# acrlabs/kube-scheduler-rs-reference

Hardware: AMD Instinct MI355X
Metric: pod x node predicate evals/s (higher is better)
Workload: dtype int64

## Files before the change

kube_scheduler_rs_reference_amd/csrc/kernels_build.hpp:

```cpp
#pragma once
#include <hip/hip_runtime.h>
#include <stdint.h>

#include "../../include/ksched.h"
#include "apply_admit.hpp"
#include "kernels_direct.hpp"
#include "tile_index.hpp"

namespace ksched {

struct BuildFitArgs {
    const int64_t *ncpu, *nmem;
    uint64_t *tables, *aux;
    const uint32_t *tile_list;
    const uint32_t *dirty;
    uint32_t n, rows, row_cpu;
};

__device__ __forceinline__ int64_t shfl_xor_key(int64_t x, uint32_t j) {
    const uint32_t lo = (uint32_t)__shfl_xor((int)(uint32_t)x, (int)j, 64), hi = (uint32_t)__shfl_xor((int)(uint32_t)((uint64_t)x >> 32), (int)j, 64);
    return (int64_t)(((uint64_t)hi << 32) | lo);
}
__device__ __forceinline__ uint32_t shfl_xor_key(uint32_t x, uint32_t j) { return (uint32_t)__shfl_xor((int)x, (int)j, 64); }

template <class K>
__device__ __forceinline__ void bitonic_sort_tile(K &kv, uint32_t &ki, K *s_key, uint16_t *s_idx, uint32_t i) {
    for (uint32_t k = 2; k <= (uint32_t)kTileNodes; k <<= 1) {
        for (uint32_t j = k >> 1; j > 0; j >>= 1) {
            K pv;
            uint32_t pi;
            if (j >= 64u) {
                s_key[i] = kv;
                s_idx[i] = (uint16_t)ki;
                __syncthreads();
                pv = s_key[i ^ j];
                pi = s_idx[i ^ j];
                __syncthreads();
            } else {
                pv = shfl_xor_key(kv, j);
                pi = shfl_xor_key(ki, j);
            }
            const bool ascending = (i & k) == 0u, lower = (i & j) == 0u;
            const bool p_less = pv < kv || (pv == kv && pi < ki);
            const bool take = (lower == ascending) ? p_less : !p_less;
            kv = take ? pv : kv;
            ki = take ? pi : ki;
        }
    }
    s_key[i] = kv;
    s_idx[i] = (uint16_t)ki;
    __syncthreads();
}

__global__ __launch_bounds__(1024) void k_build_tile_fit(const BuildFitArgs a) {
    kernarg_warm<sizeof(BuildFitArgs)>();
    __shared__ int64_t s_key[kTileNodes];
    __shared__ uint16_t s_idx[kTileNodes];
    __shared__ uint64_t s_wave[16];
    __shared__ uint64_t s_rows[kFitRows * kTileWords];
    const uint32_t tile = a.tile_list ? a.tile_list[blockIdx.x] : blockIdx.x;
    if (a.dirty && a.dirty[tile] != a.dirty[gridDim.x]) return;
    const uint32_t res = blockIdx.y;
    const int64_t *col = res == 0 ? a.ncpu : a.nmem;
    const uint32_t base = tile * kTileNodes;
    const uint32_t m = min((uint32_t)kTileNodes, a.n - base);
    const uint32_t i = threadIdx.x, lane = i & 63u, wave = i >> 6;
    int64_t kv = (i < m) ? col[base + i] : INT64_MAX;
    uint32_t ki = i;
    bitonic_sort_tile(kv, ki, s_key, s_idx, i);
    uint64_t *aux = a.aux + (size_t)tile * kAuxWords;
    {
        int64_t t;
        if (i == 0) {
            t = s_key[kTileNodes - 1];
        } else {
            const uint32_t L = 31u - (uint32_t)__builtin_clz(i), j = i - (1u << L);
            t = s_key[((2u * j + 1u) << (9u - L)) - 1u];
        }
        reinterpret_cast<int64_t *>(aux)[(size_t)res * kAuxTreeWords + i] = t;
    }
    {
        const bool live = ki < m;
        const uint32_t sub = ki / kSubNodes;
        const uint64_t x = live ? (1ull << (8u * sub)) : 0ull;
        uint64_t incl = x;
#pragma unroll
        for (uint32_t d = 1; d < 64; d <<= 1) {
            const uint32_t lo = (uint32_t)__shfl_up((int)(uint32_t)incl, d, 64), hi = (uint32_t)__shfl_up((int)(uint32_t)(incl >> 32), d, 64);
            if (lane >= d) incl += ((uint64_t)hi << 32) | lo;
        }
        if (lane == 63) s_wave[wave] = incl;
        __syncthreads();
        uint64_t before = 0, total = 0;
        for (uint32_t w = 0; w < 16; ++w) {
            const uint64_t t = s_wave[w];
            before += (w < wave) ? t : 0ull;
            total += t;
        }
        const uint64_t excl = before + incl - x;
        uint64_t *cnt = aux + 2u * kAuxTreeWords + (size_t)res * kCntEntries;
        cnt[i] = excl;
        if (i < (uint32_t)kCntEntries - (uint32_t)kTileNodes) cnt[kTileNodes + i] = total;
        __syncthreads();
        s_idx[i] = 0xFFFFu;
        __syncthreads();
        if (live) s_idx[sub * kSubNodes + (uint32_t)((excl >> (8u * sub)) & 0xFFull)] = (uint16_t)(ki & (kSubNodes - 1u));
    }
    __syncthreads();
    {
        const uint32_t sub = i >> 7, c = i & 127u;
        uint64_t *mine = s_rows + c * kTileWords + 2u * sub;
        const uint32_t node = s_idx[sub * kSubNodes + c];
        uint64_t lo = (node < 64u) ? (1ull << node) : 0ull, hi = (node >= 64u && node < 128u) ? (1ull << (node - 64u)) : 0ull;
        if (i < (uint32_t)kTileWords) s_rows[(kFitRows - 1) * kTileWords + i] = 0ull;
        auto shfl_down64 = [](uint64_t x, uint32_t d) -> uint64_t {
            const uint32_t l = (uint32_t)__shfl_down((int)(uint32_t)x, d, 64), h = (uint32_t)__shfl_down((int)(uint32_t)(x >> 32), d, 64);
            return ((uint64_t)h << 32) | l;
        };
#pragma unroll
        for (uint32_t d = 1; d < 64u; d <<= 1) {
            const uint64_t olo = shfl_down64(lo, d), ohi = shfl_down64(hi, d);
            if (lane + d < 64u) {
                lo |= olo;
                hi |= ohi;
            }
        }
        if ((c >> 6) == 1u && lane == 0) {
            s_wave[2u * sub] = lo;
            s_wave[2u * sub + 1u] = hi;
        }
        __syncthreads();
        if ((c >> 6) == 0u) {
            lo |= s_wave[2u * sub];
            hi |= s_wave[2u * sub + 1u];
        }
        mine[0] = lo;
        mine[1] = hi;
    }
    __syncthreads();
    uint64_t *T = a.tables + ((size_t)tile * a.rows + a.row_cpu + (size_t)res * kFitRows) * kTileWords;
    for (uint32_t k = i; k < (uint32_t)kFitRows * kTileWords; k += 1024u) T[k] = s_rows[k];
}

struct BuildListArgs {
    const uint32_t *nlab;
    uint8_t *lists;
    const uint32_t *tile_list;
    uint32_t n, nlist;
    uint32_t list_col[kMaxListKeys];
};
__global__ __launch_bounds__(1024) void k_build_tile_list(const BuildListArgs a) {
    kernarg_warm<sizeof(BuildListArgs)>();
    __shared__ uint32_t s_key[kTileNodes];
    __shared__ uint16_t s_idx[kTileNodes];
    const uint32_t tile = a.tile_list ? a.tile_list[blockIdx.x] : blockIdx.x, j = blockIdx.y, i = threadIdx.x;
    const uint32_t base = tile * kTileNodes;
    const uint32_t m = min((uint32_t)kTileNodes, a.n - base);
    uint32_t kv = (i < m) ? a.nlab[(size_t)a.list_col[j] * a.n + base + i] : 0u;
    uint32_t ki = i;
    bitonic_sort_tile(kv, ki, s_key, s_idx, i);
    uint8_t *L = a.lists + ((size_t)tile * a.nlist + j) * kListBytes;
    reinterpret_cast<uint32_t *>(L)[i] = kv;
    reinterpret_cast<uint16_t *>(L + kTileNodes * 4u)[i] = (uint16_t)ki;
}

struct BuildNamedArgs {
    const uint32_t *nlab;
    const uint64_t *ntaint;
    uint64_t *tables;
    const uint32_t *lab_meta;
    const uint32_t *tile_list;
    uint32_t n, rows, nkeys, ngroups, row_valid, row_taint, named_rows;
};


__global__ __launch_bounds__(1024) void k_build_tile_named(const BuildNamedArgs a) {
    kernarg_warm<sizeof(BuildNamedArgs)>();
    extern __shared__ __attribute__((aligned(16))) uint64_t s_named[];
    const uint32_t tile = a.tile_list ? a.tile_list[blockIdx.x] : blockIdx.x;
    const uint32_t base = tile * kTileNodes;
    const uint32_t m = min((uint32_t)kTileNodes, a.n - base);
    const uint32_t i = threadIdx.x, lane = i & 63u, wave = i >> 6;
    const bool live = i < m;
    const uint32_t total = a.named_rows * kTileWords;
    for (uint32_t k = i; k < total; k += 1024u) s_named[k] = 0ull;
    __syncthreads();
    {
        const uint64_t word = __ballot(live);
        if (lane == 0) s_named[a.row_valid * kTileWords + wave] = word;
    }
    if (a.ngroups) {
        const uint64_t t = (live && a.ntaint) ? a.ntaint[base + i] : 0ull;
        for (uint32_t g = 0; g < a.ngroups; ++g) {
            const uint32_t tg = (uint32_t)((t >> (4u * g)) & 15ull);
            for (uint32_t sset = 0; sset < 16; ++sset) {
                const uint64_t word = __ballot(live && (tg & ~sset) == 0u);
                if (lane == 0) s_named[(a.row_taint + 16u * g + sset) * kTileWords + wave] = word;
            }
        }
    }
    for (uint32_t k = 0; k < a.nkeys; ++k) {
        const uint32_t lb = a.lab_meta[k];
        if (lb == kLabList) continue;
        const uint32_t id = live ? a.nlab[(size_t)k * a.n + base + i] : 0u;
        if (id) atomicOr((unsigned long long *)&s_named[(size_t)(lb + id - 1u) * kTileWords + wave], 1ull << lane);
    }
    __syncthreads();
    uint64_t *T = a.tables + (size_t)tile * a.rows * kTileWords;
    for (uint32_t k = i; k < total; k += 1024u) T[k] = s_named[k];
}

constexpr uint32_t kPatchInline = 16;
struct PatchArgs {
    int64_t *ncpu, *nmem, *nrec;
    const uint32_t *idx;
    const int64_t *cpu, *mem;
    uint32_t count;
    uint32_t idx_in[kPatchInline];
    int64_t cpu_in[kPatchInline], mem_in[kPatchInline];
    uint32_t *tile_out;
    uint32_t ntiles;
    uint32_t tiles_in[kPatchInline];
};
__global__ __launch_bounds__(256) void k_patch_nodes(const PatchArgs a) {
    kernarg_warm<sizeof(PatchArgs)>();
    const uint32_t t = blockIdx.x * blockDim.x + threadIdx.x;
    if (t >= a.count) return;
    if (a.tile_out && t < a.ntiles) a.tile_out[t] = a.tiles_in[t];
    uint32_t node;
    int64_t c, m;
    if (a.idx) {
        node = a.idx[t];
        c = a.cpu[t];
        m = a.mem[t];
    } else {
        node = a.idx_in[t];
        c = a.cpu_in[t];
        m = a.mem_in[t];
    }
    a.ncpu[node] = c;
    a.nmem[node] = m;
    a.nrec[(size_t)kNodeRecWords * node] = c;
    a.nrec[(size_t)kNodeRecWords * node + 1] = m;
}

struct PatchLabelsArgs {
    uint32_t *nlab;
    uint64_t *ntaint;
    int64_t *nrec;
    const uint32_t *idx;
    const uint32_t *lab;
    const uint64_t *taints;
    uint32_t count, n, nkeys;
};
__global__ __launch_bounds__(256) void k_patch_labels(const PatchLabelsArgs a) {
    kernarg_warm<sizeof(PatchLabelsArgs)>();
    const uint32_t t = blockIdx.x * blockDim.x + threadIdx.x;
    if (t >= a.count) return;
    const uint32_t node = a.idx[t];
    uint32_t l[8];
#pragma unroll
    for (uint32_t k = 0; k < 8; ++k) l[k] = 0u;
    for (uint32_t k = 0; k < a.nkeys; ++k) {
        const uint32_t id = a.lab[(size_t)k * a.count + t];
        a.nlab[(size_t)k * a.n + node] = id;
        if (k < 8u) l[k] = id;
    }
    int64_t *r = a.nrec + (size_t)kNodeRecWords * node;
    if (a.taints) {
        const uint64_t tb = a.taints[t];
        a.ntaint[node] = tb;
        r[2] = (int64_t)tb;
    }
#pragma unroll
    for (uint32_t k = 0; k < 4; ++k) r[4 + k] = (int64_t)(((uint64_t)l[2 * k + 1] << 32) | l[2 * k]);
}

constexpr uint32_t kApplyUnclaimed = 0xFFFFFFFFu;
struct ApplyArgs {
    const int32_t *bindings;
    const int64_t *req_cpu, *req_mem;
    const uint8_t *ok;
    int32_t *status;
    uint64_t *acc;
    uint32_t *claim;
    uint8_t *ovf;
    uint32_t *dirty;
    int64_t *ncpu, *nmem, *nrec;
    uint32_t p, n, tiles, gen;
    uint32_t first_per_node, release;
    uint32_t row_lo;
    uint32_t sharded;
    const uint64_t *gathered;
    uint32_t nranks, rank;
};

__device__ __forceinline__ bool apply_eligible(const ApplyArgs &a, uint32_t i, int32_t b) {
    return b >= 0 && (uint32_t)b < a.n && (!a.ok || a.ok[i] != 0);
}

__global__ __launch_bounds__(256) void k_apply_claim(const ApplyArgs a) {
    for (uint32_t i = blockIdx.x * blockDim.x + threadIdx.x; i < a.p; i += gridDim.x * blockDim.x) {
        const int32_t b = a.bindings[i];
        if (apply_eligible(a, i, b)) atomicMin(a.claim + b, a.row_lo + i);
    }
}

__device__ __forceinline__ void acc_add(uint64_t *p, uint64_t v) {
    if (v) __hip_atomic_fetch_add(p, v, __ATOMIC_RELAXED, __HIP_MEMORY_SCOPE_AGENT);
}

__global__ __launch_bounds__(256) void k_apply_accumulate(const ApplyArgs a) {
    const uint32_t t0 = blockIdx.x * blockDim.x + threadIdx.x;
    if (t0 == 0 && !a.sharded) a.dirty[a.tiles] = a.gen;
    for (uint32_t i = t0; i < a.p; i += gridDim.x * blockDim.x) {
        const int32_t b = a.bindings[i];
        int32_t st;
        if (b < 0) {
            st = KSCHED_APPLY_UNBOUND;
        } else if ((uint32_t)b >= a.n) {
            st = KSCHED_APPLY_BAD_NODE;
        } else if (a.ok && a.ok[i] == 0) {
            st = KSCHED_APPLY_NOT_OK;
        } else if (a.first_per_node && a.claim[b] != a.row_lo + i) {
            st = KSCHED_APPLY_DEFERRED;
        } else {
// ... 364 lines not shown
```

kube_scheduler_rs_reference_amd/csrc/ksched_api.hip:

```cpp
#include "../../include/ksched.h"

#include <hip/hip_runtime.h>

#include <algorithm>
#include <cstdio>
#include <cstdlib>
#include <cstring>
#include <mutex>
#include <new>
#include <numeric>
#include <stdexcept>
#include <string>
#include <utility>
#include <vector>


#include "apply_plan.hpp"
#include "bestfit_layout.hpp"
#include "comm_rccl.hpp"
#include "eval_plan.hpp"
#include "eval_request.hpp"
#include "kernels_build.hpp"
#include "kernels_direct.hpp"
#include "kernels_fused.hpp"
#include "kernels_pick_uniform.hpp"
#include "kernels_summary.hpp"
#include "kernels_pick_spread.hpp"
#include "kernels_pick_pack.hpp"
#include "kernels_combine.hpp"
#include "kernels_combine_soft.hpp"
#include "kernels_selop.hpp"
#include "kernels_seltag.hpp"
#include "mask_alloc.hpp"
#include "merge_sort_plan.hpp"
#include "pipe_plan.hpp"
#include "snapshot_change.hpp"
#include "stream_order.hpp"
#include "tile_index.hpp"

using namespace ksched;

static_assert(kListBytes == 6144u && kTileNodes == 1024, "k_pick_bestfit_listed (kernels_direct.hpp) addresses the tile lists with these sizes");
static_assert(kChangeTileNodes == (uint32_t)kTileNodes, "snapshot_change.hpp lists the tiles an update touches");
static_assert(kApplyTileNodes == (uint32_t)kTileNodes && kApplyIdleClaim == kApplyUnclaimed, "apply_plan.hpp sizes the commit by the tile and bounds the global pod indexes by the idle claim");
static_assert(sizeof(BestfitRowsArgs::lvl_off) == 4 * kBfMaxLevels && sizeof(BfLevelsArgs::lvl_off) == 4 * kBfMaxLevels, "bestfit_layout.hpp sizes the level arrays the kernels carry");

namespace {

template <class T>
struct DevBuf {
    T *ptr = nullptr;
    size_t cap = 0;
    DevBuf() = default;
    DevBuf(DevBuf &&o) noexcept { *this = std::move(o); }
    DevBuf &operator=(DevBuf &&o) noexcept {
        std::swap(ptr, o.ptr);
        std::swap(cap, o.cap);
        return *this;
    }
    ~DevBuf() { release(); }
    void release() {
        if (ptr) (void)hipFree(ptr);
        ptr = nullptr;
        cap = 0;
    }
    hipError_t reserve(size_t n) {
        if (n <= cap) return hipSuccess;
        release();
        hipError_t e = hipMalloc((void **)&ptr, std::max<size_t>(n, 1) * sizeof(T));
        if (e == hipSuccess) cap = n;
        return e;
    }
};

struct SortScratch {
    DevBuf<int64_t> k0[2], k1[2];
    DevBuf<uint32_t> idx[2];
    bool holds(size_t n) const { return n <= k0[0].cap && n <= k0[1].cap && n <= idx[0].cap && n <= idx[1].cap; }
    hipError_t reserve(size_t n, bool second_key) {
        hipError_t e = hipSuccess;
        for (int b = 0; b < 2 && e == hipSuccess; ++b) {
            e = k0[b].reserve(n);
            if (e == hipSuccess && second_key) e = k1[b].reserve(n);
            if (e == hipSuccess) e = idx[b].reserve(n);
        }
        return e;
    }
};

struct BestfitIndex {
    DevBuf<uint32_t> bf_order, bf_rank;
    DevBuf<int64_t> bf_mem, bf_cpu;
    DevBuf<int64_t> cpu_sorted;
    DevBuf<uint32_t> by_cpu, cpurank;
    DevBuf<int64_t> samples;
    DevBuf<int64_t> levels;
    DevBuf<uint64_t> rows;
    SortScratch sort;
    DevBuf<uint32_t> handover;
    DevBuf<uint64_t> trace;
    BfOrderLayout order;
    BfRowLayout row;
    BfRotation rotation;
    bool rows_built = false;
    bool order_stale = true, rows_stale = false;

    hipError_t reserve_for(uint32_t n) {
        hipError_t e = bf_order.reserve(n);
        if (e == hipSuccess) e = bf_rank.reserve(n);
        if (e == hipSuccess) e = bf_mem.reserve(bf_searched_elems(n));
        if (e == hipSuccess) e = bf_cpu.reserve(n);
        if (e == hipSuccess) e = cpu_sorted.reserve(bf_searched_elems(n));
        return e;
    }
    void mark(Stale what) {
        if (stale_order(what)) order_stale = true;
        if (stale_rows_only(what)) rows_stale = true;
        if (what == Stale::kEverything) rows_built = false;
    }
    bool stale() const { return order_stale || rows_stale; }
};
// ... 223 lines not shown
    if (pl.carrier_waits_build)
        if (int rc = stream_wait_build(c, s)) return rc;
    if (!pl.record_callers) return KSCHED_OK;
    for (size_t i = 0; i < o.callers();) {
        if (hipEventRecord(o.caller_res(i).ev, hip_stream_of(o.caller(i))) != hipSuccess) {
            (void)hipGetLastError();
            const StreamRes gone = o.drop(i);
            (void)hipEventDestroy(gone.ev);
            continue;
        }
        HIPCHK(c, hipStreamWaitEvent(s, o.caller_res(i).ev, 0));
        ++i;
    }
    return KSCHED_OK;
}

int snapshot_end(ksched_ctx *c) {
    HIPCHK(c, hipEventRecord(c->ev_build, hip_stream_of(c->order.change_stream())));
    c->order.committed();
    return KSCHED_OK;
}

int apply_order_begin(ksched_ctx *c, hipStream_t hs) {
    if (!c->order.plan_apply(hs).change_waits_hs) return KSCHED_OK;
    if (!c->apply.ev) HIPCHK(c, hipEventCreateWithFlags(&c->apply.ev, hipEventDisableTiming));
    HIPCHK(c, hipEventRecord(c->apply.ev, hs));
    HIPCHK(c, hipStreamWaitEvent(hip_stream_of(c->order.change_stream()), c->apply.ev, 0));
    return KSCHED_OK;
}

int apply_order_end(ksched_ctx *c, hipStream_t hs) { return c->order.plan_apply(hs).hs_waits_change ? stream_wait_build(c, hs) : KSCHED_OK; }

struct SnapshotChange {
    ksched_ctx *c = nullptr;
    bool done = false;
    ~SnapshotChange() {
        if (c && !done) {
            c->have_nodes = false;
            c->apply.invalidate();
        }
    }
    int begin(ksched_ctx *ctx) {
        if (int rc = snapshot_begin(ctx)) return rc;
        c = ctx;
        return KSCHED_OK;
    }
    int stage(size_t bytes, size_t dev_bytes, uint8_t **h) {
        if (c->h_stage) HIPCHK(c, hipEventSynchronize(c->ev_stage));
        if (bytes > c->h_stage_cap) {
            if (c->h_stage) (void)hipHostFree(c->h_stage);
            c->h_stage = nullptr;
            c->h_stage_cap = 0;
            const size_t cap = std::max<size_t>(bytes + bytes / 4, 1u << 16);
            HIPCHK(c, hipHostMalloc((void **)&c->h_stage, cap, hipHostMallocDefault));
            c->h_stage_cap = cap;
        }
        *h = c->h_stage;
        HIPCHK(c, c->d_stage.reserve(dev_bytes));
        return KSCHED_OK;
    }
    int upload(size_t dev_bytes) {
        const hipStream_t s = change_stream(c);
        if (dev_bytes) HIPCHK(c, hipMemcpyAsync(c->d_stage.ptr, c->h_stage, dev_bytes, hipMemcpyHostToDevice, s));
        HIPCHK(c, hipEventRecord(c->ev_stage, s));
        return KSCHED_OK;
    }
    int commit(Stale what) {
        c->bestfit.mark(what);
        if (int rc = snapshot_end(c)) return rc;
        c->have_nodes = true;
        done = true;
        return KSCHED_OK;
    }
};


int launch_build_fit(ksched_ctx *c, const uint32_t *d_tile_list, uint32_t count, const uint32_t *d_dirty = nullptr) {
    const IndexedLayout &l = c->idx.lay;
    BuildFitArgs a{};
    a.ncpu = c->ncpu.ptr;
    a.nmem = c->nmem.ptr;
    a.tables = c->idx.d_tables;
    a.aux = c->idx.d_aux;
    a.tile_list = d_tile_list;
    a.dirty = d_tile_list ? nullptr : d_dirty;
    a.n = l.n;
    a.rows = l.rows;
    a.row_cpu = l.row_cpu;
    hipLaunchKernelGGL(k_build_tile_fit, dim3(d_tile_list ? count : l.tiles, 2), dim3(1024), 0, change_stream(c), a);
    HIPCHK(c, hipGetLastError());
    return KSCHED_OK;
}

int launch_build_lists(ksched_ctx *c, const uint32_t *d_tile_list = nullptr, uint32_t count = 0) {
    const IndexedLayout &l = c->idx.lay;
    if (l.nlist == 0) return KSCHED_OK;
    BuildListArgs a{};
    a.nlab = c->nlab.ptr;
    a.lists = c->idx.d_list;
    a.tile_list = d_tile_list;
    a.n = l.n;
    a.nlist = l.nlist;
    for (uint32_t j = 0; j < l.nlist; ++j) a.list_col[j] = l.list_col[j];
    hipLaunchKernelGGL(k_build_tile_list, dim3(d_tile_list ? count : l.tiles, l.nlist), dim3(1024), 0, change_stream(c), a);
    HIPCHK(c, hipGetLastError());
    return KSCHED_OK;
}

int launch_build_named(ksched_ctx *c, const uint32_t *d_tile_list = nullptr, uint32_t count = 0) {
    const IndexedLayout &l = c->idx.lay;
    BuildNamedArgs a{};
    a.nlab = c->nlab.ptr;
    a.ntaint = c->have_taints ? c->ntaint.ptr : nullptr;
    a.tables = c->idx.d_tables;
    a.lab_meta = c->idx.d_lab_meta;
    a.tile_list = d_tile_list;
    a.n = l.n;
    a.rows = l.rows;
    a.nkeys = l.nkeys;
    a.ngroups = l.ngroups;
    a.row_valid = l.row_valid;
    a.row_taint = l.row_taint;
    a.named_rows = l.row_cpu;
    const uint32_t lds = l.row_cpu * 128u;
    HIPCHK(c, hipFuncSetAttribute((const void *)k_build_tile_named, hipFuncAttributeMaxDynamicSharedMemorySize, (int)lds));
    hipLaunchKernelGGL(k_build_tile_named, dim3(d_tile_list ? count : l.tiles), dim3(1024), lds, change_stream(c), a);
    HIPCHK(c, hipGetLastError());
    return KSCHED_OK;
}

template <class A>
void fill_pod_operands(A &a, const ksched_ctx *c, const EvalRequest &r) {
    const bool sel = r.sel(c->nkeys);
    a.pcpu = r.pcpu;
    a.pmem = r.pmem;
    a.psel = sel ? r.psel : nullptr;
    a.ptol = r.ptol;
    a.binding = r.out_binding;
    a.p = r.p;
    a.n = c->n;
    a.nkeys = sel ? c->nkeys : 0u;
    a.do_fit = r.fit() ? 1u : 0u;
    a.do_taint = r.taint(c->have_taints) ? 1u : 0u;
}


int launch_merge_sort(ksched_ctx *c, const SortPlan &pl, const SortScratch &sc, SortBuffers io) {
    const hipStream_t s = change_stream(c);
    for (int b = 0; b < 2; ++b) {
        io.set_k0[b] = sc.k0[b].ptr;
        io.set_k1[b] = sc.k1[b].ptr;
        io.set_idx[b] = sc.idx[b].ptr;
    }
    for (uint32_t i = 0; i < pl.nsteps; ++i) {
        const SortStep &st = pl.steps[i];
        const SortPtrs ptr = sort_step_ptrs(pl, st, io);
        SortArgs q{};
        q.n = pl.n;
        q.run = st.run;
        q.k0_in = ptr.k0_in;
        q.k1_in = ptr.k1_in;
        q.idx_in = ptr.idx_in;
        q.k0_out = ptr.k0_out;
        q.k1_out = ptr.k1_out;
        q.idx_out = ptr.idx_out;
        if (st.kernel == SortKernel::kRuns) hipLaunchKernelGGL(k_sort_runs, dim3(st.grid), dim3(kSortRun), 0, s, q);
// ... 926 lines not shown
    if (count > 0 && !node_index) return KSCHED_E_INVAL;
    std::lock_guard<std::mutex> lk(c->mu);
    if (!c->have_nodes) return KSCHED_E_STATE;
    const uint32_t n = c->n, nkeys = c->nkeys;
    if (count > 0 && nkeys > 0 && !lab) return KSCHED_E_INVAL;
    for (uint32_t i = 0; i < count; ++i)
        if (node_index[i] >= n) return KSCHED_E_INVAL;
    for (size_t i = 0; i < (size_t)nkeys * count; ++i)
        if (lab[i] == KSCHED_SEL_NEVER) return KSCHED_E_INVAL;
    if (count == 0) return KSCHED_OK;
    DeviceGuard g(c->device);
    if (!g.ok) return KSCHED_E_HIP;
    fault_point(c);
    std::vector<uint32_t> keep, tiles;
    last_wins(node_index, count, keep, tiles);
    const uint32_t m = (uint32_t)keep.size();
    uint32_t lab_max[KSCHED_MAX_KEYS];
    std::copy(c->plan_lab_max, c->plan_lab_max + KSCHED_MAX_KEYS, lab_max);
    uint64_t all_taints = c->plan_taints;
    const bool holds = label_layout_holds(lab_max, &all_taints, c->idx.built, c->idx.lay.ngroups, nkeys, count, keep.data(), m, lab, taints);
    SnapshotChange chg;
    if (int rc = chg.begin(c)) return rc;
    IndexPlan plan;
    if (holds) c->plan_taints = all_taints;
    else index_plan(c, n, nkeys, lab_max, all_taints, plan);
    StageLayout f;
    const size_t o_taint = f.add<uint64_t>(taints ? m : 0), o_idx = f.add<uint32_t>(m), o_lab = f.add<uint32_t>((size_t)nkeys * m);
    const size_t o_tiles = f.add<uint32_t>(tiles.size()), b_dev = f.total, o_meta = f.add<uint32_t>(plan.indexed ? kPlanMetaWords : 0);
    uint8_t *h = nullptr;
    if (int rc = chg.stage(f.total, b_dev, &h)) return rc;
    uint64_t *ht = reinterpret_cast<uint64_t *>(h + o_taint);
    uint32_t *hi = reinterpret_cast<uint32_t *>(h + o_idx), *hl = reinterpret_cast<uint32_t *>(h + o_lab);
    for (uint32_t j = 0; j < m; ++j) {
        const uint32_t i = keep[j];
        hi[j] = node_index[i];
        if (taints) ht[j] = taints[i];
        for (uint32_t k = 0; k < nkeys; ++k) hl[(size_t)k * m + j] = lab[(size_t)k * count + i];
    }
    memcpy(h + o_tiles, tiles.data(), tiles.size() * 4);
    if (!holds)
        if (int rc = index_reserve(c, plan, h + o_meta)) return rc;
    if (int rc = chg.upload(b_dev)) return rc;
    if (taints && !c->have_taints) {
        HIPCHK(c, hipMemsetAsync(c->ntaint.ptr, 0, (size_t)n * 8, change_stream(c)));
        c->have_taints = true;
    }
    PatchLabelsArgs pa{};
    pa.nlab = c->nlab.ptr;
    pa.ntaint = taints ? c->ntaint.ptr : nullptr;
    pa.nrec = c->nrec.ptr;
    const uint8_t *d = c->d_stage.ptr;
    pa.taints = taints ? reinterpret_cast<const uint64_t *>(d + o_taint) : nullptr;
    pa.idx = reinterpret_cast<const uint32_t *>(d + o_idx);
    pa.lab = reinterpret_cast<const uint32_t *>(d + o_lab);
    pa.count = m;
    pa.n = n;
    pa.nkeys = nkeys;
    hipLaunchKernelGGL(k_patch_labels, dim3((m + 255u) / 256u), dim3(256), 0, change_stream(c), pa);
    HIPCHK(c, hipGetLastError());
    if (holds) {
        const uint32_t *d_tiles = reinterpret_cast<const uint32_t *>(d + o_tiles);
        if (int rc = launch_build_named(c, d_tiles, (uint32_t)tiles.size())) return rc;
        if (int rc = launch_build_lists(c, d_tiles, (uint32_t)tiles.size())) return rc;
    } else {
        if (int rc = index_build(c, plan, false, nullptr, nullptr, nullptr, nullptr)) return rc;
    }
    return chg.commit(Stale::kLabels);
} KSCHED_ABI_CATCH(c)

int ksched_update_nodes(ksched_ctx *c, uint32_t count, const uint32_t *node_index, const int64_t *cpu, const int64_t *mem) try {
    if (!c) return KSCHED_E_INVAL;
    if (count > 0 && (!node_index || !cpu || !mem)) return KSCHED_E_INVAL;
    std::lock_guard<std::mutex> lk(c->mu);
    if (!c->have_nodes) return KSCHED_E_STATE;
    for (uint32_t i = 0; i < count; ++i)
        if (node_index[i] >= c->n) return KSCHED_E_INVAL;
    if (count == 0) return KSCHED_OK;
    DeviceGuard g(c->device);
    if (!g.ok) return KSCHED_E_HIP;
    fault_point(c);
    std::vector<uint32_t> keep, tiles;
    last_wins(node_index, count, keep, tiles);
    const uint32_t m = (uint32_t)keep.size();
    SnapshotChange chg;
    if (int rc = chg.begin(c)) return rc;
    PatchArgs pa{};
    pa.ncpu = c->ncpu.ptr;
    pa.nmem = c->nmem.ptr;
    pa.nrec = c->nrec.ptr;
    pa.count = m;
    const uint32_t *d_tiles = nullptr;
    if (m <= kPatchInline && tiles.size() <= kPatchInline) {
        for (uint32_t j = 0; j < m; ++j) {
            pa.idx_in[j] = node_index[keep[j]];
            pa.cpu_in[j] = cpu[keep[j]];
            pa.mem_in[j] = mem[keep[j]];
        }
    } else {
        StageLayout f;
        const size_t o_idx = f.add<uint32_t>(m), o_cpu = f.add<int64_t>(m), o_mem = f.add<int64_t>(m), o_tiles = f.add<uint32_t>(tiles.size());
        uint8_t *h = nullptr;
        if (int rc = chg.stage(f.total, f.total, &h)) return rc;
        uint32_t *hi = reinterpret_cast<uint32_t *>(h + o_idx);
        int64_t *hc = reinterpret_cast<int64_t *>(h + o_cpu), *hm = reinterpret_cast<int64_t *>(h + o_mem);
        for (uint32_t j = 0; j < m; ++j) {
            hi[j] = node_index[keep[j]];
            hc[j] = cpu[keep[j]];
            hm[j] = mem[keep[j]];
        }
        memcpy(h + o_tiles, tiles.data(), tiles.size() * 4);
        if (int rc = chg.upload(f.total)) return rc;
        const uint8_t *d = c->d_stage.ptr;
        pa.idx = reinterpret_cast<const uint32_t *>(d + o_idx);
        pa.cpu = reinterpret_cast<const int64_t *>(d + o_cpu);
        pa.mem = reinterpret_cast<const int64_t *>(d + o_mem);
        d_tiles = reinterpret_cast<const uint32_t *>(d + o_tiles);
    }
    if (c->idx.built && !d_tiles) {
        HIPCHK(c, c->d_stage.reserve(kPatchInline * 4));
        pa.tile_out = reinterpret_cast<uint32_t *>(c->d_stage.ptr);
        pa.ntiles = (uint32_t)tiles.size();
        for (size_t j = 0; j < tiles.size(); ++j) pa.tiles_in[j] = tiles[j];
        d_tiles = pa.tile_out;
    }
    hipLaunchKernelGGL(k_patch_nodes, dim3((m + 255u) / 256u), dim3(256), 0, change_stream(c), pa);
    HIPCHK(c, hipGetLastError());
    if (c->idx.built) {
        if (int rc = launch_build_fit(c, d_tiles, (uint32_t)tiles.size())) return rc;
    }
    return chg.commit(Stale::kAvailable);
} KSCHED_ABI_CATCH(c)

int ksched_read_nodes(ksched_ctx *c, uint32_t first, uint32_t count, int64_t *out_cpu, int64_t *out_mem) try {
    if (!c) return KSCHED_E_INVAL;
    if (count > 0 && (!out_cpu || !out_mem)) return KSCHED_E_INVAL;
    std::lock_guard<std::mutex> lk(c->mu);
    if (!c->have_nodes) return KSCHED_E_STATE;
    if ((uint64_t)first + count > c->n) return KSCHED_E_INVAL;
    if (count == 0) return KSCHED_OK;
    DeviceGuard g(c->device);
    if (!g.ok) return KSCHED_E_HIP;
    fault_point(c);
    HIPCHK(c, hipEventSynchronize(c->ev_build));
    HIPCHK(c, hipMemcpy(out_cpu, c->ncpu.ptr + first, (size_t)count * 8, hipMemcpyDeviceToHost));
    HIPCHK(c, hipMemcpy(out_mem, c->nmem.ptr + first, (size_t)count * 8, hipMemcpyDeviceToHost));
    return KSCHED_OK;
} KSCHED_ABI_CATCH(c)

int ksched_eval_device_pitched(ksched_ctx *c, uint32_t p, const int64_t *pcpu, const int64_t *pmem, const uint32_t *psel,
                               const uint64_t *ptol, const uint32_t *samples, uint32_t attempts, uint32_t flags,
                               uint64_t *out_feas, uint64_t *out_fit, int32_t *out_binding, uint32_t mask_pitch_words,
                               void *hip_stream) try {
    if (!c) return KSCHED_E_INVAL;
    std::lock_guard<std::mutex> lk(c->mu);
    if (!c->have_nodes) return KSCHED_E_STATE;
    const EvalRequest r{p, pcpu, pmem, psel, ptol, samples, attempts, flags, out_feas, out_fit, out_binding, mask_pitch_words, (hipStream_t)hip_stream};
    int rc = check_eval_args(r, true);
    if (rc) return rc;
    if (mask_pitch_words < c->W) return KSCHED_E_INVAL;
    DeviceGuard g(c->device);
    if (!g.ok) return KSCHED_E_HIP;
    return eval_on_device(c, r);
} KSCHED_ABI_CATCH(c)

int ksched_eval_device(ksched_ctx *c, uint32_t p, const int64_t *pcpu, const int64_t *pmem, const uint32_t *psel,
                       const uint64_t *ptol, const uint32_t *samples, uint32_t attempts, uint32_t flags,
                       uint64_t *out_feas, uint64_t *out_fit, int32_t *out_binding, void *hip_stream) try {
    return ksched_eval_device_pitched(c, p, pcpu, pmem, psel, ptol, samples, attempts, flags, out_feas, out_fit, out_binding,
                                      ksched_mask_words(ksched_num_nodes(c)), hip_stream);
} KSCHED_ABI_CATCH(c)

uint32_t ksched_mask_pitch(uint32_t n_nodes) { return (ksched_mask_words(n_nodes) + 15u) & ~15u; }

struct ksched_pipe {
    ksched_ctx *ctx = nullptr;
    uint32_t depth = 0;
    std::vector<hipStream_t> streams;
    std::vector<hipEvent_t> mask_done, pick_done;
    std::vector<PipeSlot> slots;
};

int ksched_pipe_create(ksched_ctx *c, uint32_t depth, ksched_pipe **out) try {
    if (!c || !out || depth == 0 || depth > 64) return KSCHED_E_INVAL;
    *out = nullptr;
    DeviceGuard g(c->device);
    if (!g.ok) return KSCHED_E_HIP;
    ksched_pipe *q = new (std::nothrow) ksched_pipe();
    if (!q) return KSCHED_E_NOMEM;
    q->ctx = c;
    q->depth = depth;
    q->slots.assign(depth, PipeSlot{});
    bool ok = true;
    for (int i = 0; ok && i <= kPipePickStream; ++i) {
        hipStream_t s = nullptr;
        ok = hipStreamCreateWithFlags(&s, hipStreamNonBlocking) == hipSuccess;
        if (ok) q->streams.push_back(s);
    }
    for (uint32_t i = 0; ok && i < 2 * depth; ++i) {
        hipEvent_t e;
        ok = hipEventCreateWithFlags(&e, hipEventDisableTiming) == hipSuccess;
        if (ok) (i < depth ? q->mask_done : q->pick_done).push_back(e);
    }
    if (!ok) {
        ksched_pipe_destroy(q);
        return KSCHED_E_HIP;
    }
    *out = q;
    return KSCHED_OK;
} KSCHED_ABI_CATCH(c)

void ksched_pipe_destroy(ksched_pipe *q) try {
// ... 1060 lines not shown
```

kube_scheduler_rs_reference_amd/csrc/tile_index.hpp:

```cpp
#pragma once
#include <hip/hip_runtime.h>
#include <stdint.h>

#include <algorithm>
#include <climits>
#include <numeric>
#include <vector>

#include "../../include/ksched.h"

namespace ksched {

constexpr int kTileWords = 16;
constexpr int kTileNodes = kTileWords * 64;
constexpr int kSubNodes = 128;
constexpr int kSubTiles = kTileNodes / kSubNodes;
constexpr int kFitRows = kSubNodes + 1;
constexpr int kCntEntries = kTileNodes + 2;
constexpr int kIdxMaxKeys = 32;
constexpr int kIdxMaxGroups = 16;
constexpr uint32_t kLdsBudget = 160u * 1024u;
constexpr uint32_t kAuxTreeWords = kTileNodes;
constexpr uint32_t kAuxWords = 2u * kAuxTreeWords + 2u * kCntEntries;
constexpr uint32_t kLdsNonRowBytesMax = kAuxWords * 8u + 1024u * 40u;
constexpr uint32_t kMaxListKeys = 2;
constexpr uint32_t kListBytes = kTileNodes * 4u + kTileNodes * 2u;
constexpr uint32_t kListRecBytes = 8u;
constexpr uint32_t kLabList = 0xFFFFFFFFu;
constexpr uint32_t lds_non_row_bytes(uint32_t nlist) { return kLdsNonRowBytesMax + nlist * kListBytes + (nlist ? 1024u * kListRecBytes : 0u); }

struct IndexedLayout {
    uint32_t n, W, tiles, rows, nkeys, ngroups;
    uint32_t row_zero, row_valid;
    uint32_t row_cpu, row_mem;
    uint32_t row_taint;
    uint32_t lab_base[kIdxMaxKeys];
    uint32_t lab_max[kIdxMaxKeys];
    uint32_t nlist;
    uint32_t list_col[kMaxListKeys];
};

struct IndexedSnapshot {
    bool built = false;
    IndexedLayout lay{};
    uint64_t *d_tables = nullptr;
    uint64_t *d_aux = nullptr;
    uint32_t *d_lab_meta = nullptr;
    uint8_t *d_list = nullptr;
    size_t aux_cap = 0, tables_cap = 0, list_cap = 0;
};

inline void indexed_release(IndexedSnapshot &s) {
    if (s.d_aux) (void)hipFree(s.d_aux);
    if (s.d_tables) (void)hipFree(s.d_tables);
    if (s.d_lab_meta) (void)hipFree(s.d_lab_meta);
    if (s.d_list) (void)hipFree(s.d_list);
    s = IndexedSnapshot{};
}

inline uint32_t indexed_lds_bytes(const IndexedLayout &l) { return l.rows * 128u; }

inline void eytzinger_from_sorted(const int64_t *sorted, int64_t *tree) {
    tree[0] = sorted[kTileNodes - 1];
    for (uint32_t level = 0; level < 10; ++level)
        for (uint32_t j = 0; j < (1u << level); ++j) tree[(1u << level) + j] = sorted[((2u * j + 1u) << (9u - level)) - 1u];
}

inline void index_tile_fit(const IndexedLayout &l, uint32_t t, const int64_t *cpu, const int64_t *mem, uint64_t *T, uint64_t *aux) {
    const uint32_t base = t * kTileNodes;
    const uint32_t m = std::min<uint32_t>(kTileNodes, l.n - base);
    std::fill(T + (size_t)l.row_cpu * kTileWords, T + (size_t)(l.row_cpu + 2 * kFitRows) * kTileWords, 0ull);
    auto setbit = [&](uint32_t row, uint32_t local) { T[(size_t)row * kTileWords + (local >> 6)] |= 1ull << (local & 63u); };
    uint32_t ord[kTileNodes];
    int64_t sorted[kTileNodes];
    for (int res = 0; res < 2; ++res) {
        const int64_t *v = res == 0 ? cpu : mem;
        const uint32_t row0 = res == 0 ? l.row_cpu : l.row_mem;
        int64_t *tree = reinterpret_cast<int64_t *>(aux) + (size_t)res * kAuxTreeWords;
        uint64_t *cnt = aux + 2u * kAuxTreeWords + (size_t)res * kCntEntries;
        std::fill(sorted, sorted + kTileNodes, INT64_MAX);
        std::iota(ord, ord + m, 0u);
        std::stable_sort(ord, ord + m, [&](uint32_t a, uint32_t b) { return v[base + a] < v[base + b]; });
        uint64_t packed = 0;
        uint32_t seen[kSubTiles] = {};
        for (uint32_t pos = 0; pos < m; ++pos) {
            cnt[pos] = packed;
            const uint32_t local = ord[pos], s = local / kSubNodes;
            sorted[pos] = v[base + local];
            const uint32_t lr = seen[s]++;
            for (uint32_t c = 0; c <= lr; ++c) setbit(row0 + c, local);
            packed += 1ull << (8u * s);
        }
        for (uint32_t r = m; r < (uint32_t)kCntEntries; ++r) cnt[r] = packed;
        eytzinger_from_sorted(sorted, tree);
    }
}

inline bool indexed_plan(IndexedLayout &l, uint32_t n, uint32_t nkeys, const uint32_t *lab_max, uint64_t all_taints, const char **why) {
    if (n == 0) {
        *why = "no nodes";
        return false;
    }
    if (nkeys > kIdxMaxKeys) {
        *why = "more label keys than the bitmap index holds";
        return false;
    }
    l = IndexedLayout{};
    l.n = n;
    l.W = (n + 63u) / 64u;
    l.tiles = (n + kTileNodes - 1) / kTileNodes;
    l.nkeys = nkeys;
    l.ngroups = all_taints ? (uint32_t)((64 - __builtin_clzll(all_taints)) + 3) / 4 : 0;
    uint32_t r = 0;
    l.row_zero = r++;
    l.row_valid = r++;
    l.row_taint = r; r += 16 * l.ngroups;
    for (uint32_t k = 0; k < nkeys; ++k) l.lab_max[k] = lab_max[k];
    bool is_list[kIdxMaxKeys] = {};
    for (;;) {
        uint64_t label_rows = 0;
        for (uint32_t k = 0; k < nkeys; ++k)
            if (!is_list[k]) label_rows += (uint64_t)lab_max[k] + 1u;
        const uint64_t lds = (r + label_rows + 2u * kFitRows) * 128u + lds_non_row_bytes(l.nlist);
        if (lds <= kLdsBudget && (r + label_rows) * 128u <= 65536u) break;
        if (l.nlist == kMaxListKeys) {
            *why = "more than two high-cardinality label keys: their (key, value) rows exceed the LDS budget of the fused kernel";
            return false;
        }
        uint32_t big = nkeys;
        for (uint32_t k = 0; k < nkeys; ++k)
            if (!is_list[k] && (big == nkeys || lab_max[k] > lab_max[big])) big = k;
        if (big == nkeys) {
            *why = "the fit rows alone exceed the LDS budget";
            return false;
        }
        is_list[big] = true;
        ++l.nlist;
    }
    {
        uint32_t j = 0;
        for (uint32_t k = 0; k < nkeys; ++k)
            if (is_list[k]) l.list_col[j++] = k;
    }
    for (uint32_t k = 0; k < nkeys; ++k) {
        if (is_list[k]) {
            l.lab_base[k] = kLabList;
            continue;
        }
        l.lab_base[k] = r;
        r += l.lab_max[k] + 1u;
    }
    l.row_cpu = r; r += kFitRows;
    l.row_mem = r; r += kFitRows;
    l.rows = r;
    return true;
}

inline hipError_t indexed_reserve(IndexedSnapshot &s, const IndexedLayout &l) {
    hipError_t e;
    const size_t aux_words = (size_t)l.tiles * kAuxWords, tab_words = (size_t)l.tiles * l.rows * kTileWords;
    if (aux_words > s.aux_cap) {
        if (s.d_aux) (void)hipFree(s.d_aux);
        s.d_aux = nullptr;
        s.aux_cap = 0;
        if ((e = hipMalloc((void **)&s.d_aux, aux_words * 8)) != hipSuccess) return e;
        s.aux_cap = aux_words;
    }
    if (tab_words > s.tables_cap) {
        if (s.d_tables) (void)hipFree(s.d_tables);
        s.d_tables = nullptr;
        s.tables_cap = 0;
        if ((e = hipMalloc((void **)&s.d_tables, tab_words * 8)) != hipSuccess) return e;
        s.tables_cap = tab_words;
    }
    if (!s.d_lab_meta && (e = hipMalloc((void **)&s.d_lab_meta, 72 * sizeof(uint32_t))) != hipSuccess) return e;
    const size_t list_bytes = (size_t)l.tiles * l.nlist * kListBytes;
    if (list_bytes > s.list_cap) {
        if (s.d_list) (void)hipFree(s.d_list);
        s.d_list = nullptr;
        s.list_cap = 0;
        if ((e = hipMalloc((void **)&s.d_list, list_bytes)) != hipSuccess) return e;
        s.list_cap = list_bytes;
    }
    return hipSuccess;
}

inline void indexed_meta(const IndexedLayout &l, uint32_t meta[72]) {
    for (int k = 0; k < 72; ++k) meta[k] = 0;
    for (int k = 0; k < 32; ++k) {
        meta[k] = l.lab_base[k];
        meta[32 + k] = l.lab_max[k];
    }
}

inline hipError_t indexed_build_host(IndexedSnapshot &s, const IndexedLayout &l, const int64_t *cpu, const int64_t *mem, const uint32_t *lab,
                                     const uint64_t *taints, hipStream_t stream) {
    const uint32_t n = l.n, nkeys = l.nkeys;
    const size_t tile_words = (size_t)l.rows * kTileWords;
    std::vector<uint64_t> tab((size_t)l.tiles * tile_words, 0ull);
    std::vector<uint64_t> aux((size_t)l.tiles * kAuxWords, 0ull);
    std::vector<uint8_t> lists((size_t)l.tiles * l.nlist * kListBytes, 0);
    for (uint32_t t = 0; t < l.tiles; ++t) {
        const uint32_t base = t * kTileNodes;
        const uint32_t m = std::min<uint32_t>(kTileNodes, n - base);
        uint64_t *T = tab.data() + (size_t)t * tile_words;
        auto setbit = [&](uint32_t row, uint32_t local) { T[(size_t)row * kTileWords + (local >> 6)] |= 1ull << (local & 63u); };
        for (uint32_t i = 0; i < m; ++i) setbit(l.row_valid, i);
        index_tile_fit(l, t, cpu, mem, T, aux.data() + (size_t)t * kAuxWords);
        for (uint32_t k = 0; k < nkeys; ++k) {
            if (l.lab_base[k] == kLabList) continue;
            for (uint32_t i = 0; i < m; ++i) {
                const uint32_t id = lab[(size_t)k * n + base + i];
                if (id) setbit(l.lab_base[k] + id - 1, i);
            }
        }
        for (uint32_t j = 0; j < l.nlist; ++j) {
            const uint32_t k = l.list_col[j];
            uint32_t ord[kTileNodes], val[kTileNodes];
            for (uint32_t i = 0; i < (uint32_t)kTileNodes; ++i) {
                ord[i] = i;
                val[i] = i < m ? lab[(size_t)k * n + base + i] : 0u;
            }
            std::stable_sort(ord, ord + kTileNodes, [&](uint32_t x, uint32_t y) { return val[x] < val[y]; });
            uint8_t *L = lists.data() + ((size_t)t * l.nlist + j) * kListBytes;
            uint32_t *vals = reinterpret_cast<uint32_t *>(L);
            uint16_t *nodes = reinterpret_cast<uint16_t *>(L + kTileNodes * 4u);
            for (uint32_t i = 0; i < (uint32_t)kTileNodes; ++i) {
                vals[i] = val[ord[i]];
                nodes[i] = (uint16_t)ord[i];
            }
        }
        for (uint32_t g = 0; g < l.ngroups; ++g)
            for (uint32_t i = 0; i < m; ++i) {
                const uint32_t tg = (uint32_t)((taints[base + i] >> (4 * g)) & 15ull);
                for (uint32_t sub = 0; sub < 16; ++sub)
                    if ((tg & ~sub) == 0) setbit(l.row_taint + 16 * g + sub, i);
            }
    }
    hipError_t e;
    if ((e = hipMemcpyAsync(s.d_aux, aux.data(), aux.size() * 8, hipMemcpyHostToDevice, stream)) != hipSuccess) return e;
    if ((e = hipMemcpyAsync(s.d_tables, tab.data(), tab.size() * 8, hipMemcpyHostToDevice, stream)) != hipSuccess) return e;
    if (!lists.empty() && (e = hipMemcpyAsync(s.d_list, lists.data(), lists.size(), hipMemcpyHostToDevice, stream)) != hipSuccess) return e;
    if ((e = hipStreamSynchronize(stream)) != hipSuccess) return e;
    return hipSuccess;
}

typedef unsigned long long u64x2 __attribute__((ext_vector_type(2)));

}
```

Baseline: 27430 billion.

## Fuse small node updates into one kernel with incremental re-sort from stored order

```diff
diff --git a/kube_scheduler_rs_reference_amd/csrc/kernels_build.hpp b/kube_scheduler_rs_reference_amd/csrc/kernels_build.hpp
--- a/kube_scheduler_rs_reference_amd/csrc/kernels_build.hpp
+++ b/kube_scheduler_rs_reference_amd/csrc/kernels_build.hpp
@@ -6,12 +6,14 @@
 #include "apply_admit.hpp"
 #include "kernels_direct.hpp"
 #include "tile_index.hpp"
+#include "update_plan.hpp"
 
 namespace ksched {
 
 struct BuildFitArgs {
     const int64_t *ncpu, *nmem;
     uint64_t *tables, *aux;
+    uint16_t *order;
     const uint32_t *tile_list;
     const uint32_t *dirty;
     uint32_t n, rows, row_cpu;
@@ -52,22 +54,15 @@
     __syncthreads();
 }
 
-__global__ __launch_bounds__(1024) void k_build_tile_fit(const BuildFitArgs a) {
-    kernarg_warm<sizeof(BuildFitArgs)>();
-    __shared__ int64_t s_key[kTileNodes];
-    __shared__ uint16_t s_idx[kTileNodes];
-    __shared__ uint64_t s_wave[16];
-    __shared__ uint64_t s_rows[kFitRows * kTileWords];
-    const uint32_t tile = a.tile_list ? a.tile_list[blockIdx.x] : blockIdx.x;
-    if (a.dirty && a.dirty[tile] != a.dirty[gridDim.x]) return;
-    const uint32_t res = blockIdx.y;
-    const int64_t *col = res == 0 ? a.ncpu : a.nmem;
-    const uint32_t base = tile * kTileNodes;
-    const uint32_t m = min((uint32_t)kTileNodes, a.n - base);
+struct FitTileOut {
+    uint64_t *tables, *aux;
+    uint16_t *order;
+    uint32_t rows, row_cpu;
+};
+__device__ __forceinline__ void build_tile_fit_body(const uint32_t ki, uint32_t tile, uint32_t res, uint32_t m, const FitTileOut a, int64_t *s_key,
+                                                    uint16_t *s_idx, uint64_t *s_wave, uint64_t *s_rows) {
     const uint32_t i = threadIdx.x, lane = i & 63u, wave = i >> 6;
-    int64_t kv = (i < m) ? col[base + i] : INT64_MAX;
-    uint32_t ki = i;
-    bitonic_sort_tile(kv, ki, s_key, s_idx, i);
+    a.order[((size_t)tile * 2u + res) * kTileNodes + i] = (uint16_t)ki;
     uint64_t *aux = a.aux + (size_t)tile * kAuxWords;
     {
         int64_t t;
@@ -142,6 +137,25 @@
     for (uint32_t k = i; k < (uint32_t)kFitRows * kTileWords; k += 1024u) T[k] = s_rows[k];
 }
 
+__global__ __launch_bounds__(1024) void k_build_tile_fit(const BuildFitArgs a) {
+    kernarg_warm<sizeof(BuildFitArgs)>();
+    __shared__ int64_t s_key[kTileNodes];
+    __shared__ uint16_t s_idx[kTileNodes];
+    __shared__ uint64_t s_wave[16];
+    __shared__ uint64_t s_rows[kFitRows * kTileWords];
+    const uint32_t tile = a.tile_list ? a.tile_list[blockIdx.x] : blockIdx.x;
+    if (a.dirty && a.dirty[tile] != a.dirty[gridDim.x]) return;
+    const uint32_t res = blockIdx.y;
+    const int64_t *col = res == 0 ? a.ncpu : a.nmem;
+    const uint32_t base = tile * kTileNodes;
+    const uint32_t m = min((uint32_t)kTileNodes, a.n - base);
+    const uint32_t i = threadIdx.x;
+    int64_t kv = (i < m) ? col[base + i] : INT64_MAX;
+    uint32_t ki = i;
+    bitonic_sort_tile(kv, ki, s_key, s_idx, i);
+    build_tile_fit_body(ki, tile, res, m, FitTileOut{a.tables, a.aux, a.order, a.rows, a.row_cpu}, s_key, s_idx, s_wave, s_rows);
+}
+
 struct BuildListArgs {
     const uint32_t *nlab;
     uint8_t *lists;
@@ -211,6 +225,7 @@
 }
 
 constexpr uint32_t kPatchInline = 16;
+static_assert(kPatchInline == kUpdateInline, "update_plan.hpp decides with the same bound");
 struct PatchArgs {
     int64_t *ncpu, *nmem, *nrec;
     const uint32_t *idx;
@@ -218,15 +233,11 @@
     uint32_t count;
     uint32_t idx_in[kPatchInline];
     int64_t cpu_in[kPatchInline], mem_in[kPatchInline];
-    uint32_t *tile_out;
-    uint32_t ntiles;
-    uint32_t tiles_in[kPatchInline];
 };
 __global__ __launch_bounds__(256) void k_patch_nodes(const PatchArgs a) {
     kernarg_warm<sizeof(PatchArgs)>();
     const uint32_t t = blockIdx.x * blockDim.x + threadIdx.x;
     if (t >= a.count) return;
-    if (a.tile_out && t < a.ntiles) a.tile_out[t] = a.tiles_in[t];
     uint32_t node;
     int64_t c, m;
     if (a.idx) {
@@ -242,6 +253,71 @@
     a.nmem[node] = m;
     a.nrec[(size_t)kNodeRecWords * node] = c;
     a.nrec[(size_t)kNodeRecWords * node + 1] = m;
+}
+
+struct UpdateTilesArgs {
+    int64_t *ncpu, *nmem, *nrec;
+    uint64_t *tables, *aux;
+    uint16_t *order;
+    uint32_t n, rows, row_cpu;
+    UpdateEntries e;
+};
+static_assert(sizeof(UpdateTilesArgs) <= 512, "kernarg_warm touches eight lines at most");
+__global__ __launch_bounds__(1024) void k_update_tiles_fit(const UpdateTilesArgs a) {
+    kernarg_warm<sizeof(UpdateTilesArgs)>();
+    __shared__ int64_t s_key[kTileNodes];
+    __shared__ uint16_t s_idx[kTileNodes];
+    __shared__ uint64_t s_wave[16];
+    __shared__ uint64_t s_rows[kFitRows * kTileWords];
+    const uint32_t tile = a.e.tiles[blockIdx.x];
+    const uint32_t res = blockIdx.y;
+    int64_t *col = res == 0 ? a.ncpu : a.nmem;
+    const uint32_t base = tile * kTileNodes;
+    const uint32_t m = min((uint32_t)kTileNodes, a.n - base);
+    const uint32_t i = threadIdx.x, lane = i & 63u, wave = i >> 6;
+    uint32_t ki = a.order[((size_t)tile * 2u + res) * kTileNodes + i] & (uint32_t)(kTileNodes - 1);
+    int64_t kv = (ki < m) ? col[base + ki] : INT64_MAX;
+    const uint32_t count = min(a.e.count, kPatchInline);
+    uint32_t mine = kPatchInline;
+    for (uint32_t j = 0; j < count; ++j) {
+        const uint32_t node = a.e.idx[j];
+        const int64_t v = res == 0 ? a.e.cpu[j] : a.e.mem[j];
+        if (node == base + ki) {
+            kv = v;
+            mine = j;
+            col[node] = v;
+            a.nrec[(size_t)kNodeRecWords * node + res] = v;
+        }
+    }
+    const bool patched = mine < kPatchInline;
+    uint32_t *s_cnt = reinterpret_cast<uint32_t *>(s_rows);
+    const uint64_t ub = __ballot(!patched);
+    const uint32_t ulow = (uint32_t)__popcll(ub & ((1ull << lane) - 1ull));
+    if (lane == 0) s_cnt[kPatchInline * 16u + wave] = (uint32_t)__popcll(ub);
+    uint32_t shift = 0;
+    for (uint32_t j = 0; j < count; ++j) {
+        const uint32_t node = a.e.idx[j];
+        if (node / kTileNodes != tile) continue;
+        const int64_t v = res == 0 ? a.e.cpu[j] : a.e.mem[j];
+        const uint32_t nj = node - base;
+        const bool below = v < kv || (v == kv && nj < ki);
+        shift += below ? 1u : 0u;
+        const uint64_t b = __ballot(!patched && !below);
+        if (lane == 0) s_cnt[j * 16u + wave] = (uint32_t)__popcll(b);
+    }
+    __syncthreads();
+    uint32_t pos = shift;
+    if (patched) {
+        for (uint32_t w = 0; w < 16u; ++w) pos += s_cnt[mine * 16u + w];
+    } else {
+        pos += ulow;
+        for (uint32_t w = 0; w < 16u; ++w) pos += (w < wave) ? s_cnt[kPatchInline * 16u + w] : 0u;
+    }
+    s_key[pos] = kv;
+    s_idx[pos] = (uint16_t)ki;
+    __syncthreads();
+    ki = s_idx[i];
+    build_tile_fit_body(ki, tile, res, m, FitTileOut{a.tables, a.aux, a.order, a.rows, a.row_cpu}, s_key, s_idx, s_wave, s_rows);
 }
 
 struct PatchLabelsArgs {
diff --git a/kube_scheduler_rs_reference_amd/csrc/ksched_api.hip b/kube_scheduler_rs_reference_amd/csrc/ksched_api.hip
--- a/kube_scheduler_rs_reference_amd/csrc/ksched_api.hip
+++ b/kube_scheduler_rs_reference_amd/csrc/ksched_api.hip
@@ -37,6 +37,7 @@
 #include "snapshot_change.hpp"
 #include "stream_order.hpp"
 #include "tile_index.hpp"
+#include "update_plan.hpp"
 
 using namespace ksched;
 
@@ -426,6 +427,7 @@
     a.nmem = c->nmem.ptr;
     a.tables = c->idx.d_tables;
     a.aux = c->idx.d_aux;
+    a.order = c->idx.d_order;
     a.tile_list = d_tile_list;
     a.dirty = d_tile_list ? nullptr : d_dirty;
     a.n = l.n;
@@ -1518,20 +1520,38 @@
     std::vector<uint32_t> keep, tiles;
     last_wins(node_index, count, keep, tiles);
     const uint32_t m = (uint32_t)keep.size();
+    const UpdatePlan plan = plan_update_nodes(m, tiles.size(), c->idx.built);
+    UpdateEntries e;
+    if (!plan.stage) fill_update_entries(e, node_index, cpu, mem, keep.data(), m, tiles.data(), tiles.size());
     SnapshotChange chg;
     if (int rc = chg.begin(c)) return rc;
+    if (plan.path == UpdatePath::kFused) {
+        const IndexedLayout &l = c->idx.lay;
+        UpdateTilesArgs ua{};
+        ua.ncpu = c->ncpu.ptr;
+        ua.nmem = c->nmem.ptr;
+        ua.nrec = c->nrec.ptr;
+        ua.tables = c->idx.d_tables;
+        ua.aux = c->idx.d_aux;
+        ua.order = c->idx.d_order;
+        ua.n = l.n;
+        ua.rows = l.rows;
+        ua.row_cpu = l.row_cpu;
+        ua.e = e;
+        hipLaunchKernelGGL(k_update_tiles_fit, dim3(plan.fused.x, plan.fused.y), dim3(plan.fused.block), 0, change_stream(c), ua);
+        HIPCHK(c, hipGetLastError());
+        return chg.commit(Stale::kAvailable);
+    }
     PatchArgs pa{};
     pa.ncpu = c->ncpu.ptr;
     pa.nmem = c->nmem.ptr;
     pa.nrec = c->nrec.ptr;
     pa.count = m;
     const uint32_t *d_tiles = nullptr;
-    if (m <= kPatchInline && tiles.size() <= kPatchInline) {
-        for (uint32_t j = 0; j < m; ++j) {
-            pa.idx_in[j] = node_index[keep[j]];
-            pa.cpu_in[j] = cpu[keep[j]];
-            pa.mem_in[j] = mem[keep[j]];
-        }
+    if (!plan.stage) {
+        memcpy(pa.idx_in, e.idx, sizeof(pa.idx_in));
+        memcpy(pa.cpu_in, e.cpu, sizeof(pa.cpu_in));
+        memcpy(pa.mem_in, e.mem, sizeof(pa.mem_in));
     } else {
         StageLayout f;
         const size_t o_idx = f.add<uint32_t>(m), o_cpu = f.add<int64_t>(m), o_mem = f.add<int64_t>(m), o_tiles = f.add<uint32_t>(tiles.size());
@@ -1552,17 +1572,10 @@
         pa.mem = reinterpret_cast<const int64_t *>(d + o_mem);
         d_tiles = reinterpret_cast<const uint32_t *>(d + o_tiles);
     }
-    if (c->idx.built && !d_tiles) {
-        HIPCHK(c, c->d_stage.reserve(kPatchInline * 4));
-        pa.tile_out = reinterpret_cast<uint32_t *>(c->d_stage.ptr);
-        pa.ntiles = (uint32_t)tiles.size();
-        for (size_t j = 0; j < tiles.size(); ++j) pa.tiles_in[j] = tiles[j];
-        d_tiles = pa.tile_out;
-    }
-    hipLaunchKernelGGL(k_patch_nodes, dim3((m + 255u) / 256u), dim3(256), 0, change_stream(c), pa);
+    hipLaunchKernelGGL(k_patch_nodes, dim3(plan.patch.x), dim3(plan.patch.block), 0, change_stream(c), pa);
     HIPCHK(c, hipGetLastError());
-    if (c->idx.built) {
-        if (int rc = launch_build_fit(c, d_tiles, (uint32_t)tiles.size())) return rc;
+    if (plan.reindex.x) {
+        if (int rc = launch_build_fit(c, d_tiles, plan.reindex.x)) return rc;
     }
     return chg.commit(Stale::kAvailable);
 } KSCHED_ABI_CATCH(c)
diff --git a/kube_scheduler_rs_reference_amd/csrc/tile_index.hpp b/kube_scheduler_rs_reference_amd/csrc/tile_index.hpp
--- a/kube_scheduler_rs_reference_amd/csrc/tile_index.hpp
+++ b/kube_scheduler_rs_reference_amd/csrc/tile_index.hpp
@@ -47,7 +47,8 @@
     uint64_t *d_aux = nullptr;
     uint32_t *d_lab_meta = nullptr;
     uint8_t *d_list = nullptr;
-    size_t aux_cap = 0, tables_cap = 0, list_cap = 0;
+    uint16_t *d_order = nullptr;
+    size_t aux_cap = 0, tables_cap = 0, list_cap = 0, order_cap = 0;
 };
 
 inline void indexed_release(IndexedSnapshot &s) {
@@ -55,6 +56,7 @@
     if (s.d_tables) (void)hipFree(s.d_tables);
     if (s.d_lab_meta) (void)hipFree(s.d_lab_meta);
     if (s.d_list) (void)hipFree(s.d_list);
+    if (s.d_order) (void)hipFree(s.d_order);
     s = IndexedSnapshot{};
 }
 
@@ -66,7 +68,8 @@
         for (uint32_t j = 0; j < (1u << level); ++j) tree[(1u << level) + j] = sorted[((2u * j + 1u) << (9u - level)) - 1u];
 }
 
-inline void index_tile_fit(const IndexedLayout &l, uint32_t t, const int64_t *cpu, const int64_t *mem, uint64_t *T, uint64_t *aux) {
+inline void index_tile_fit(const IndexedLayout &l, uint32_t t, const int64_t *cpu, const int64_t *mem, uint64_t *T, uint64_t *aux,
+                           uint16_t *order = nullptr) {
     const uint32_t base = t * kTileNodes;
     const uint32_t m = std::min<uint32_t>(kTileNodes, l.n - base);
     std::fill(T + (size_t)l.row_cpu * kTileWords, T + (size_t)(l.row_cpu + 2 * kFitRows) * kTileWords, 0ull);
@@ -93,6 +96,8 @@
         }
         for (uint32_t r = m; r < (uint32_t)kCntEntries; ++r) cnt[r] = packed;
         eytzinger_from_sorted(sorted, tree);
+        if (order)
+            for (uint32_t pos = 0; pos < (uint32_t)kTileNodes; ++pos) order[(size_t)res * kTileNodes + pos] = (uint16_t)(pos < m ? ord[pos] : pos);
     }
 }
 
@@ -182,6 +187,14 @@
         if ((e = hipMalloc((void **)&s.d_list, list_bytes)) != hipSuccess) return e;
         s.list_cap = list_bytes;
     }
+    const size_t order_elems = (size_t)l.tiles * 2u * kTileNodes;
+    if (order_elems > s.order_cap) {
+        if (s.d_order) (void)hipFree(s.d_order);
+        s.d_order = nullptr;
+        s.order_cap = 0;
+        if ((e = hipMalloc((void **)&s.d_order, order_elems * 2)) != hipSuccess) return e;
+        s.order_cap = order_elems;
+    }
     return hipSuccess;
 }
 
@@ -200,13 +213,14 @@
     std::vector<uint64_t> tab((size_t)l.tiles * tile_words, 0ull);
     std::vector<uint64_t> aux((size_t)l.tiles * kAuxWords, 0ull);
     std::vector<uint8_t> lists((size_t)l.tiles * l.nlist * kListBytes, 0);
+    std::vector<uint16_t> order((size_t)l.tiles * 2u * kTileNodes, 0);
     for (uint32_t t = 0; t < l.tiles; ++t) {
         const uint32_t base = t * kTileNodes;
         const uint32_t m = std::min<uint32_t>(kTileNodes, n - base);
         uint64_t *T = tab.data() + (size_t)t * tile_words;
         auto setbit = [&](uint32_t row, uint32_t local) { T[(size_t)row * kTileWords + (local >> 6)] |= 1ull << (local & 63u); };
         for (uint32_t i = 0; i < m; ++i) setbit(l.row_valid, i);
-        index_tile_fit(l, t, cpu, mem, T, aux.data() + (size_t)t * kAuxWords);
+        index_tile_fit(l, t, cpu, mem, T, aux.data() + (size_t)t * kAuxWords, order.data() + (size_t)t * 2u * kTileNodes);
         for (uint32_t k = 0; k < nkeys; ++k) {
             if (l.lab_base[k] == kLabList) continue;
             for (uint32_t i = 0; i < m; ++i) {
@@ -241,6 +255,7 @@
     if ((e = hipMemcpyAsync(s.d_aux, aux.data(), aux.size() * 8, hipMemcpyHostToDevice, stream)) != hipSuccess) return e;
     if ((e = hipMemcpyAsync(s.d_tables, tab.data(), tab.size() * 8, hipMemcpyHostToDevice, stream)) != hipSuccess) return e;
     if (!lists.empty() && (e = hipMemcpyAsync(s.d_list, lists.data(), lists.size(), hipMemcpyHostToDevice, stream)) != hipSuccess) return e;
+    if ((e = hipMemcpyAsync(s.d_order, order.data(), order.size() * 2, hipMemcpyHostToDevice, stream)) != hipSuccess) return e;
     if ((e = hipStreamSynchronize(stream)) != hipSuccess) return e;
     return hipSuccess;
 }
diff --git a/kube_scheduler_rs_reference_amd/csrc/update_plan.hpp b/kube_scheduler_rs_reference_amd/csrc/update_plan.hpp
--- /dev/null
+++ b/kube_scheduler_rs_reference_amd/csrc/update_plan.hpp
@@ -0,0 +1,63 @@
+#pragma once
+
+#include <cstddef>
+#include <cstdint>
+
+namespace ksched {
+
+constexpr uint32_t kUpdateInline = 16;
+constexpr uint32_t kUpdateTileBlock = 1024;
+constexpr uint32_t kUpdatePatchBlock = 256;
+
+enum class UpdatePath : uint8_t { kNothing, kFused, kPatchInline, kStaged };
+
+struct UpdateGrid {
+    uint32_t x = 0, y = 0, block = 0;
+};
+struct UpdatePlan {
+    UpdatePath path = UpdatePath::kNothing;
+    bool stage = false;
+    UpdateGrid fused;
+    UpdateGrid patch;
+    UpdateGrid reindex;
+    uint32_t launches() const { return (fused.x ? 1u : 0u) + (patch.x ? 1u : 0u) + (reindex.x ? 1u : 0u); }
+};
+
+inline UpdatePlan plan_update_nodes(size_t kept, size_t tiles, bool index_built) {
+    UpdatePlan pl;
+    if (kept == 0) return pl;
+    const bool small = kept <= kUpdateInline && tiles <= kUpdateInline;
+    if (small && index_built) {
+        pl.path = UpdatePath::kFused;
+        pl.fused = UpdateGrid{(uint32_t)tiles, 2u, kUpdateTileBlock};
+        return pl;
+    }
+    pl.path = small ? UpdatePath::kPatchInline : UpdatePath::kStaged;
+    pl.stage = !small;
+    pl.patch = UpdateGrid{(uint32_t)((kept + kUpdatePatchBlock - 1u) / kUpdatePatchBlock), 1u, kUpdatePatchBlock};
+    if (index_built) pl.reindex = UpdateGrid{(uint32_t)tiles, 2u, kUpdateTileBlock};
+    return pl;
+}
+
+struct UpdateEntries {
+    uint32_t count = 0, ntiles = 0;
+    uint32_t idx[kUpdateInline] = {};
+    int64_t cpu[kUpdateInline] = {}, mem[kUpdateInline] = {};
+    uint32_t tiles[kUpdateInline] = {};
+};
+inline bool fill_update_entries(UpdateEntries &e, const uint32_t *node_index, const int64_t *cpu, const int64_t *mem, const uint32_t *keep, size_t kept,
+                                const uint32_t *tiles, size_t ntiles) {
+    if (kept > kUpdateInline || ntiles > kUpdateInline) return false;
+    e = UpdateEntries{};
+    e.count = (uint32_t)kept;
+    e.ntiles = (uint32_t)ntiles;
+    for (size_t j = 0; j < kept; ++j) {
+        e.idx[j] = node_index[keep[j]];
+        e.cpu[j] = cpu[keep[j]];
+        e.mem[j] = mem[keep[j]];
+    }
+    for (size_t j = 0; j < ntiles; ++j) e.tiles[j] = tiles[j];
+    return true;
+}
+
+}
```

New measurement: 24720 billion. 9.9% lower.
